# ACDSLab/MPPI-Generic

Measured on AMD Instinct MI355X. Metric: MPPI iters/sec (KxT rollouts), higher is better.
Workload: dtype f32; 1 GPU; Cartpole (CartpoleDynamics + CartpoleQuadraticCost, examples/cartpole_example.cu config) VanillaMPPI optimisation iteration, T=100, dt=0.02, lambda=0.25, sigma=5, Philox noise fused in the rollout kernel, K=16384 rollouts per GPU; rollouts_per_gpu=16384, global_rollouts=16384, parallelism=K-sharded x1, exchange=none

## Files before the change

### include/mppi_amd/dynamics/cartpole/cartpole_dynamics.hpp

```cpp
#ifndef MPPI_AMD_CARTPOLE_DYNAMICS_HPP_
#define MPPI_AMD_CARTPOLE_DYNAMICS_HPP_

#include "mppi_amd/plugin/dynamics.hpp"

struct CartpoleDynamicsParams : public DynamicsParams
{
  enum class StateIndex : int
  {
    POS_X = 0,
    VEL_X,
    THETA,
    THETA_DOT,
    NUM_STATES
  };
  enum class ControlIndex : int
  {
    FORCE = 0,
    NUM_CONTROLS
  };
  enum class OutputIndex : int
  {
    POS_X = 0,
    VEL_X,
    THETA,
    THETA_DOT,
    NUM_OUTPUTS
  };
  float cart_mass = 1.0f;
  float pole_mass = 1.0f;
  float pole_length = 1.0f;

  CartpoleDynamicsParams() = default;
  CartpoleDynamicsParams(float cart_mass, float pole_mass, float pole_length)
    : cart_mass(cart_mass), pole_mass(pole_mass), pole_length(pole_length){};
};

using namespace MPPI_internal;

class CartpoleDynamics : public Dynamics<CartpoleDynamics, CartpoleDynamicsParams>
{
public:
  static constexpr bool MPPI_BARRIER_FREE_STEP = true;
  using PARENT_CLASS = Dynamics<CartpoleDynamics, CartpoleDynamicsParams>;
  CartpoleDynamics(float cart_mass = 1.0f, float pole_mass = 1.0f, float pole_length = 1.0f, hipStream_t stream = 0)
    : PARENT_CLASS(stream)
  {
    this->params_ = CartpoleDynamicsParams(cart_mass, pole_mass, pole_length);
  }

  static const char* getDynamicsModelName()
  {
    return "Cartpole Model";
  }
  __host__ __device__ float getCartMass()
  {
    return this->params_.cart_mass;
  };
  __host__ __device__ float getPoleMass()
  {
    return this->params_.pole_mass;
  };
  __host__ __device__ float getPoleLength()
  {
    return this->params_.pole_length;
  };
  __host__ __device__ float getGravity()
  {
    return gravity_;
  }

  __device__ inline void computeDynamics(float* state, float* control, float* state_der, float* theta = nullptr)
  {
    float theta_n = angle_utils::normalizeAngleBounded(state[2]);
    float sin_theta, cos_theta;
    mppi::det::sincos(theta_n, &sin_theta, &cos_theta);
    float theta_dot = state[3];
    float force = control[0];
    float m_c = this->params_.cart_mass;
    float m_p = this->params_.pole_mass;
    float l_p = this->params_.pole_length;

    state_der[0] = state[1];
    const float den = m_c + m_p * SQ(sin_theta);
    float r_x, r_th;
    mppi::det::rcp_benign2(den, l_p * den, &r_x, &r_th);
    state_der[1] = r_x * (force + m_p * sin_theta * (l_p * SQ(theta_dot) + gravity_ * cos_theta));
    state_der[2] = theta_dot;
    state_der[3] =
        r_th *
        (-force * cos_theta - m_p * l_p * SQ(theta_dot) * cos_theta * sin_theta - (m_c + m_p) * gravity_ * sin_theta);
  }

protected:
  const float gravity_ = 9.81;
};

#endif
```

### include/mppi_amd/engine/rollout_pipeline_kernel.hpp

```cpp
#ifndef MPPI_AMD_ROLLOUT_PIPELINE_KERNEL_HPP_
#define MPPI_AMD_ROLLOUT_PIPELINE_KERNEL_HPP_

#include <type_traits>
#include "rollout_kernel.hpp"
#include "merge_wave.hpp"
#include "kernarg_view.hpp"

namespace mppi
{
namespace kernels
{
constexpr int PIPE_ROLES = 3;
__host__ __device__ constexpr int pipeRingSteps(int output_dim)
{
  return output_dim <= 8 ? 32 : (output_dim <= 16 ? 16 : 8);
}

template <class DYN_T, class COST_T, class SAMPLING_T>
__host__ inline size_t pipelineSharedBytes(const DYN_T& dyn, const COST_T& cost, const SAMPLING_T& smp, int bz,
                                           bool fold_z = false)
{
  const int slots = fold_z ? 64 : 64 * bz;
  const int rings = fold_z ? 1 : bz;
  size_t n = 0;
  n += calcClassSharedMemSize(&dyn, slots);
  n += calcClassSharedMemSize(&cost, slots);
  n += calcClassSharedMemSize(&smp, slots);
  n += sizeof(float) * 2 * math::nearest_multiple_4(slots);
  n += sizeof(float) * (size_t)rings * pipeRingSteps(DYN_T::OUTPUT_DIM) *
       (DYN_T::OUTPUT_DIM + (smp.rows_global_d_ ? DYN_T::CONTROL_DIM : 0)) * 64;
  n += sizeof(int) * 4 * 4 * rings;
  n += sizeof(float) * math::nearest_multiple_4(smp.params_.num_timesteps * DYN_T::CONTROL_DIM);
  return n;
}

typedef volatile __attribute__((address_space(3))) int* lds_counter_t;
typedef int pipe_int4 __attribute__((ext_vector_type(4)));
typedef volatile __attribute__((address_space(3))) pipe_int4* lds_counter4_t;

__device__ inline void pipeWait(lds_counter_t ctr, const int need, int& cached)
{
  if (cached >= need)
    return;
  int v = __builtin_amdgcn_readfirstlane(*ctr);
  while (v < need)
  {
    __builtin_amdgcn_s_sleep(1);
    v = __builtin_amdgcn_readfirstlane(*ctr);
  }
  cached = v;
  __builtin_amdgcn_fence(__ATOMIC_ACQUIRE, "workgroup");
}
__device__ inline void pipePublish(lds_counter_t ctr, const int value, const int lane)
{
  __builtin_amdgcn_fence(__ATOMIC_RELEASE, "workgroup");
  if (lane == 0)
    *ctr = value;
}
__device__ inline void pipePublishLds(lds_counter_t ctr, const int value, const int lane)
{
  asm volatile("" ::: "memory");
  if (lane == 0)
    *ctr = value;
  asm volatile("" ::: "memory");
}
#if defined(MPPI_PIPE_TIMING)
constexpr int PIPE_TIMING_BLOCKS = 256, PIPE_TIMING_WAVES = 24, PIPE_TIMING_SLOTS = 8;
static __device__ unsigned long long g_pipe_timing[PIPE_TIMING_BLOCKS * PIPE_TIMING_WAVES * PIPE_TIMING_SLOTS];
struct PipeTimer
{
  unsigned long long acc[PIPE_TIMING_SLOTS] = {};
  unsigned long long t0 = 0;
  __device__ inline void start()
  {
    t0 = __builtin_amdgcn_s_memtime();
  }
  __device__ inline void stop(const int slot)
  {
    const unsigned long long t1 = __builtin_amdgcn_s_memtime();
    acc[slot] += t1 - t0;
    t0 = t1;
  }
  __device__ inline void trip(const int block, const int kind, const int trip_idx, const int lane, const unsigned long long v) const
  {
    if (block < PIPE_TIMING_BLOCKS && lane == 0 && trip_idx < 4 * PIPE_TIMING_SLOTS && kind < 5)
      g_pipe_timing[(block * PIPE_TIMING_WAVES + 4 + 4 * kind) * PIPE_TIMING_SLOTS + trip_idx] = v;
  }
  __device__ inline void flush(const int block, const int wave, const int lane) const
  {
    if (block < PIPE_TIMING_BLOCKS && wave < PIPE_TIMING_WAVES && lane == 0)
      for (int i = 0; i < PIPE_TIMING_SLOTS; i++)
        g_pipe_timing[(block * PIPE_TIMING_WAVES + wave) * PIPE_TIMING_SLOTS + i] = acc[i];
  }
};
#define PIPE_T(x) x
#else
#define PIPE_T(x)
#endif

constexpr int PIPE_SAMPLERS = 2;
__host__ __device__ constexpr int pipelineBlockX(int bz, bool fold_z)
{
  return (bz == 1 || fold_z) ? 64 * (2 + PIPE_SAMPLERS) : 64 * PIPE_ROLES;
}

template <class DYN_T, class COST_T, class SAMPLING_T, int BZ, bool DRAW_IN_LOOP, bool FOLD_Z = false, bool ROWS_HBM = false,
          bool STREAM_MERGE = false>
__global__ void __launch_bounds__(pipelineBlockX(BZ, FOLD_Z) * (FOLD_Z ? 1 : BZ))
    rolloutPipelineKernel(DYN_T dynamics_obj, COST_T costs_obj, SAMPLING_T sampling_obj, const RolloutArgs args)
{
  static_assert(!STREAM_MERGE || (BZ == 1 && !FOLD_Z && !ROWS_HBM && DRAW_IN_LOOP), "STREAM_MERGE: one system, plain draw, LDS rows");
  static_assert(!FOLD_Z || 64 % BZ == 0, "systems must divide the wave");
  constexpr int BX = FOLD_Z ? 64 / BZ : 64;
  constexpr int WZ = FOLD_Z ? 1 : BZ;
  constexpr bool PAIR_DRAW = FOLD_Z && DRAW_IN_LOOP && BZ == 2 && DYN_T::CONTROL_DIM == 2;
  constexpr int WX = pipelineBlockX(BZ, FOLD_Z);
  constexpr int NS = WX / 64 - 2;
  __builtin_assume(__builtin_amdgcn_workgroup_size_x() == WX);
  __builtin_assume(__builtin_amdgcn_workgroup_size_y() == 1);
  __builtin_assume(__builtin_amdgcn_workgroup_size_z() == WZ);
  __builtin_assume(__builtin_amdgcn_workitem_id_x() < WX);
  __builtin_assume(__builtin_amdgcn_workitem_id_y() == 0);
  __builtin_assume(__builtin_amdgcn_workitem_id_z() < WZ);

  PIPE_T(PipeTimer tm; tm.start(); const unsigned long long t_entry = wall_clock64();)
  DYN_T* dynamics = &dynamics_obj;
  COST_T* costs = &costs_obj;
  SAMPLING_T* sampling = &sampling_obj;
  constexpr int S = DYN_T::STATE_DIM, C = DYN_T::CONTROL_DIM, O = DYN_T::OUTPUT_DIM;
  constexpr int PIPE_RING = pipeRingSteps(O);
  constexpr int SLOTS = BX * BZ;
  constexpr int NTHREADS = WX * WZ;
  constexpr bool SMP_CONSTRAINS = !DYN_T::CONSTRAINTS_DEPEND_ON_STATE;

  const int tid_x = (int)__builtin_amdgcn_workitem_id_x();
  const int wave_x = __builtin_amdgcn_readfirstlane(tid_x >> 6);
  const int role = wave_x < PIPE_ROLES ? wave_x : 0;
  const int smp_id = wave_x < PIPE_ROLES ? 0 : wave_x - PIPE_ROLES + 1;
  const int lane = tid_x & 63;
  const int thread_idx = FOLD_Z ? lane % BX : lane;
  const int thread_idz = FOLD_Z ? lane / BX : (int)__builtin_amdgcn_workitem_id_z();
  const int ring_z = FOLD_Z ? 0 : thread_idz;
  const int block_idx = (int)blockIdx.x;
  const int global_idx = BX * block_idx + thread_idx;
  const int shared_idx = BX * thread_idz + thread_idx;
  const int distribution_idx = thread_idz;
  sampling->setNoiseStream(distribution_idx);
  const int tid_flat = tid_x + WX * ring_z;
  const int num_timesteps = args.num_timesteps;
  const int num_rollouts = args.num_rollouts;
  const float dt = args.dt;
  const bool valid = global_idx < num_rollouts;
  const int nrows = min(BX, num_rollouts - BX * block_idx);

  extern __shared__ __attribute__((aligned(16))) char smem_raw[];
  float* theta_s_shared = reinterpret_cast<float*>(smem_raw);
  float* theta_c_shared = theta_s_shared + calcClassSharedMemSize(dynamics, SLOTS) / (int)sizeof(float);
  float* theta_d_lds = theta_c_shared + calcClassSharedMemSize(costs, SLOTS) / (int)sizeof(float);
  float* theta_d_shared = theta_d_lds;
  if constexpr (ROWS_HBM)
  {
    theta_d_shared = sampling->blockRows(theta_d_lds, (int)blockIdx.x, SLOTS);
    sampling->setStagingBase(theta_d_lds);
  }
  constexpr int F = O + (ROWS_HBM ? C : 0);
  float* cost_s = theta_d_lds + calcClassSharedMemSize(sampling, SLOTS) / (int)sizeof(float);
  float* w_s = cost_s + math::nearest_multiple_4(SLOTS);
  float* ring_all = w_s + math::nearest_multiple_4(SLOTS);
  float* ring = ring_all + (size_t)ring_z * PIPE_RING * F * 64;
  lds_counter_t counters =
      (lds_counter_t)(reinterpret_cast<int*>(ring_all + (size_t)WZ * PIPE_RING * F * 64) + 16 * ring_z);
  float* mean_row_s = ring_all + (size_t)WZ * PIPE_RING * F * 64 + 16 * WZ;
  lds_counter_t smp_prog = counters + 0;
  lds_counter_t smp_prog1 = counters + 1;
  lds_counter_t cost_prog = counters + 2;
  lds_counter_t dyn_prog = counters + 4;
  static_assert(NS <= 2, "one spare counter");

  sampling->setThreadMapping(shared_idx, BX, BZ);

  float x[S], x_next[S], xdot[S], u[C], y[O];
  int crash_status = 0;
#pragma unroll
  for (int i = 0; i < S; i++)
  {
    x[i] = 0.0f;
    xdot[i] = 0.0f;
    x_next[i] = 0.0f;
  }
#pragma unroll
  for (int i = 0; i < C; i++)
    u[i] = 0.0f;
#pragma unroll
  for (int i = 0; i < O; i++)
    y[i] = 0.0f;
  constexpr int SMP_STEPS = 4;
  constexpr int TRIP_COLS = SMP_STEPS * C;
  constexpr int TRIP_GROUPS = TRIP_COLS / MERGE_COLS;
  typedef float merge_f4 __attribute__((ext_vector_type(4)));
  MergeTails mt;
  merge_f4 vq[STREAM_MERGE ? TRIP_GROUPS : 1][MERGE_LANE_RECORDS];
  typedef float merge_f2 __attribute__((ext_vector_type(2)));
  merge_f2 tailq[MERGE_LANE_RECORDS];
  const int TC_all = num_timesteps * C;
  auto load_trip_columns = [&](const int t) {
    if constexpr (STREAM_MERGE)
    {
      static_assert(MERGE_COLS == 4, "the transposed copy is laid out in column quads");
#pragma unroll
      for (int g = 0; g < TRIP_GROUPS; g++)
      {
        const int col0 = t * C + MERGE_COLS * g;
#pragma unroll
        for (int i = 0; i < MERGE_LANE_RECORDS; i++)
        {
          const int b = lane + 64 * i;
          const bool ok = b < args.prev_num_records && col0 < TC_all;
          vq[g][i] = *reinterpret_cast<const merge_f4*>(args.prev_records_t_d +
                                                        ((size_t)(ok ? col0 >> 2 : 0) * args.prev_num_records + (ok ? b : 0)) * 4);
        }
      }
    }
  };
  auto sampler_trip = [&](const int t, auto first_trip) {
    constexpr int QUADS = C;
    float zq[4 * QUADS];
    if (DRAW_IN_LOOP)
    {
#pragma unroll
      for (int q = 0; q < QUADS; q++)
        sampling->drawQuad(global_idx, t * C / 4 + q, &zq[4 * q]);
    }
    PIPE_T(if (decltype(first_trip)::value && smp_id == 0) tm.trip(block_idx, 4, 1, lane, __builtin_amdgcn_s_memtime() - tm.t0);)
    float mu[TRIP_COLS];
    if constexpr (STREAM_MERGE)
    {
      if constexpr (decltype(first_trip)::value)
      {
#pragma unroll
        for (int q = 0; q < 4 * QUADS; q++)
          asm volatile("" : "+v"(zq[q]));
        __builtin_amdgcn_sched_barrier(0);
        float rho_b[MERGE_LANE_RECORDS], eta_b[MERGE_LANE_RECORDS], eta2_b[MERGE_LANE_RECORDS];
#pragma unroll
        for (int i = 0; i < MERGE_LANE_RECORDS; i++)
        {
          const bool ok = lane + 64 * i < args.prev_num_records;
          rho_b[i] = ok ? tailq[i].x : INFINITY;
          eta_b[i] = ok ? tailq[i].y : 0.0f;
          eta2_b[i] = 0.0f;
        }
        mergeTails<false>(rho_b, eta_b, eta2_b, (float)(1.0 / (double)args.lambda), mt);
      }
      PIPE_T(if (decltype(first_trip)::value && smp_id == 0) tm.trip(block_idx, 4, 2, lane, __builtin_amdgcn_s_memtime() - tm.t0);)
#pragma unroll
      for (int g = 0; g < TRIP_GROUPS; g++)
      {
        float v[MERGE_LANE_RECORDS][MERGE_COLS], tot[MERGE_COLS];
#pragma unroll
        for (int i = 0; i < MERGE_LANE_RECORDS; i++)
        {
          const bool ok = lane + 64 * i < args.prev_num_records;
          v[i][0] = ok ? vq[g][i].x : 0.0f;
          v[i][1] = ok ? vq[g][i].y : 0.0f;
          v[i][2] = ok ? vq[g][i].z : 0.0f;
          v[i][3] = ok ? vq[g][i].w : 0.0f;
        }
        mergeColumns(mt.s, v, tot);
#pragma unroll
        for (int c = 0; c < MERGE_COLS; c++)
        {
          mu[MERGE_COLS * g + c] = tot[c] / mt.eta_f;
          if (t * C + MERGE_COLS * g + c < TC_all)
            mean_row_s[t * C + MERGE_COLS * g + c] = mu[MERGE_COLS * g + c];
        }
      }
      PIPE_T(if (decltype(first_trip)::value && smp_id == 0) tm.trip(block_idx, 4, 3, lane, __builtin_amdgcn_s_memtime() - tm.t0);)
      load_trip_columns(t + SMP_STEPS * NS);
    }
#pragma unroll
    for (int s2 = 0; s2 < SMP_STEPS; s2++)
    {
      if (t + s2 < num_timesteps)
      {
        if constexpr (STREAM_MERGE)
          sampling->template shapeControlSampleMean<FOLD_Z>(global_idx, t + s2, distribution_idx, &zq[s2 * C], &mu[s2 * C], u);
        else if (DRAW_IN_LOOP)
          sampling->template shapeControlSample<FOLD_Z>(global_idx, t + s2, distribution_idx, &zq[s2 * C], u);
        else
          sampling->template readControlSample<FOLD_Z>(global_idx, t + s2, distribution_idx, u, theta_d_shared, 1, 0, y);
        if (SMP_CONSTRAINS)
          dynamics->enforceConstraints(x, u);
        sampling->writeControlSample(global_idx, t + s2, distribution_idx, u, theta_d_shared, 1, 0, y);
      }
    }
    PIPE_T(if (decltype(first_trip)::value && smp_id == 0) tm.trip(block_idx, 4, 4, lane, __builtin_amdgcn_s_memtime() - tm.t0);)
  };
  constexpr bool EARLY_FIRST_TRIP = DRAW_IN_LOOP && !PAIR_DRAW;
  static_assert(!STREAM_MERGE || EARLY_FIRST_TRIP, "STREAM_MERGE: the record tails are merged inside the early first trip");
  if constexpr (STREAM_MERGE)
  {
    if (role == 0)
    {
      const float* tails_t = args.prev_records_t_d + (size_t)TC_all * args.prev_num_records;
#pragma unroll
      for (int i = 0; i < MERGE_LANE_RECORDS; i++)
      {
        const int b = lane + 64 * i;
        tailq[i] = *reinterpret_cast<const merge_f2*>(tails_t + 2 * (b < args.prev_num_records ? b : 0));
      }
      load_trip_columns(SMP_STEPS * smp_id);
      asm volatile("" ::: "memory");
      PIPE_T(if (smp_id == 0) tm.trip(block_idx, 4, 0, lane, __builtin_amdgcn_s_memtime() - tm.t0);)
    }
  }
  if (EARLY_FIRST_TRIP && role == 0 && SMP_STEPS * smp_id < num_timesteps)
    sampler_trip(SMP_STEPS * smp_id, std::true_type{});
#pragma unroll
  for (int i = 0; i < S; i++)
    x[i] = args.init_x_d[S * thread_idz + i];

  if (lane == 0 && wave_x == 0)
  {
    *smp_prog = 0;
    *dyn_prog = 0;
    *cost_prog = 0;
    *smp_prog1 = 0;
  }
  __syncthreads();

  dynamics->initializeDynamics(x, u, y, theta_s_shared, 0.0f, dt);
  sampling->initializeDistributions(y, 0.0f, dt, theta_d_shared);
  costs->initializeCosts(y, u, theta_c_shared, 0.0f, dt);
  __syncthreads();

  float running_cost = 0.0f;
  float* row = sampling->sampleRow(theta_d_shared, shared_idx);
  PIPE_T(tm.stop(3);)

  if (role == 0 && PAIR_DRAW)
  {
    constexpr int STEPS = 8 / C;
    lds_counter_t my_prog = smp_id == 0 ? smp_prog : smp_prog1;
    for (int t = STEPS * smp_id; t < num_timesteps; t += STEPS * NS)
    {
      float zq[4], e[8];
      if (sampling->independentNoise())
      {
        sampling->drawQuad(global_idx, t * C / 4, &e[0]);
        sampling->drawQuad(global_idx, t * C / 4 + 1, &e[4]);
      }
      else
      {
        sampling->drawQuad(global_idx, t * C / 4 + thread_idz, zq);
#pragma unroll
        for (int l = 0; l < 4; l++)
        {
          const unsigned v = __float_as_uint(zq[l]);
          auto r = __builtin_amdgcn_permlane32_swap(v, v, false, false);
          e[l] = __uint_as_float(r[0]);
          e[4 + l] = __uint_as_float(r[1]);
        }
      }
#pragma unroll
      for (int s2 = 0; s2 < STEPS; s2++)
      {
        if (t + s2 < num_timesteps)
        {
          sampling->template shapeControlSample<FOLD_Z>(global_idx, t + s2, distribution_idx, &e[s2 * C], u);
          if (SMP_CONSTRAINS)
            dynamics->enforceConstraints(x, u);
          sampling->writeControlSample(global_idx, t + s2, distribution_idx, u, theta_d_shared, 1, 0, y);
        }
      }
      pipePublish(my_prog, min(t + STEPS, num_timesteps), lane);
    }
  }
  else if (role == 0)
  {
    constexpr int STEPS = SMP_STEPS;
    lds_counter_t my_prog = smp_id == 0 ? smp_prog : smp_prog1;
    auto publish = [&](const int value) {
      if constexpr (ROWS_HBM)
        pipePublish(my_prog, value, lane);
      else
        pipePublishLds(my_prog, value, lane);
    };
    int t = STEPS * smp_id;
    if (EARLY_FIRST_TRIP && t < num_timesteps)
    {
      publish(min(t + STEPS, num_timesteps));
      t += STEPS * NS;
    }
    for (; t < num_timesteps; t += STEPS * NS)
    {
      sampler_trip(t, std::false_type{});
      publish(min(t + STEPS, num_timesteps));
      PIPE_T(if (smp_id == 0) { const unsigned long long ts0 = tm.t0; tm.stop(0); tm.trip(block_idx, 3, t / (STEPS * NS), lane, tm.t0 - ts0); })
    }
    PIPE_T(tm.stop(0);)
  }
  else if (role == 1)
  {
    auto dyn_step = [&](float* xc, float* xn, int t, const float* u_in) {
#pragma unroll
      for (int i = 0; i < C; i++)
        u[i] = u_in[i];
      if (!SMP_CONSTRAINS)
      {
        dynamics->enforceConstraints(xc, u);
#pragma unroll
        for (int i = 0; i < C; i++)
          row[t * C + i] = u[i];
      }
      dynamics->step(xc, xn, xdot, u, y, theta_s_shared, t, dt);
      float* slot = ring + (size_t)(t % PIPE_RING) * F * 64 + lane;
#pragma unroll
      for (int i = 0; i < O; i++)
        slot[i * 64] = y[i];
      if constexpr (ROWS_HBM)
      {
#pragma unroll
        for (int i = 0; i < C; i++)
          slot[(O + i) * 64] = u[i];
      }
    };
    int seen_smp = 0, seen_smp1 = 0, seen_cost = 0;
    int t = 0;
    pipe_int4 ahead = { 0, 0, 0, 0 };
    auto look_ahead = [&]() { ahead = *(lds_counter4_t)counters; };
    auto need = [&](lds_counter_t ctr, int& cached, const int ahead_value, const int n) {
      if (cached >= n)
        return;
      cached = max(cached, __builtin_amdgcn_readfirstlane(ahead_value));
      if (cached >= n)
        __builtin_amdgcn_fence(__ATOMIC_ACQUIRE, "workgroup");
      else
        pipeWait(ctr, n, cached);
    };
    auto wait_trip = [&](const int tp, const int n) {
      if (NS == 2 && (tp & 4))
        need(smp_prog1, seen_smp1, ahead.y, n);
      else
        need(smp_prog, seen_smp, ahead.x, n);
    };
    auto wait_ring = [&](const int n) { need(cost_prog, seen_cost, ahead.z, n); };
    float unext[4 * C];
    auto prefetch = [&](const int tp) {
      if (tp < num_timesteps)
      {
        wait_trip(tp, min(tp + 4, num_timesteps));
#pragma unroll
        for (int j = 0; j < 4 * C; j++)
          unext[j] = (tp * C + j < num_timesteps * C) ? row[tp * C + j] : 0.0f;
      }
    };
    if constexpr (ROWS_HBM)
      prefetch(0);
    if constexpr (!ROWS_HBM && NS == 2)
    {
      for (; t + 7 < num_timesteps; t += 8)
      {
        need(smp_prog, seen_smp, ahead.x, t + 4);
        need(smp_prog1, seen_smp1, ahead.y, t + 8);
        PIPE_T(const unsigned long long tw0 = tm.t0; tm.stop(1); tm.trip(block_idx, 0, t / 8, lane, tm.t0 - tw0);)
        wait_ring(t + 8 - PIPE_RING);
        PIPE_T(const unsigned long long tw1 = tm.t0; tm.stop(2); tm.trip(block_idx, 1, t / 8, lane, tm.t0 - tw1);)
        float ubuf[8 * C];
#pragma unroll
        for (int j = 0; j < 8 * C; j++)
          ubuf[j] = row[t * C + j];
        dyn_step(x, x_next, t, &ubuf[0]);
        dyn_step(x_next, x, t + 1, &ubuf[C]);
        dyn_step(x, x_next, t + 2, &ubuf[2 * C]);
        dyn_step(x_next, x, t + 3, &ubuf[3 * C]);
        dyn_step(x, x_next, t + 4, &ubuf[4 * C]);
        dyn_step(x_next, x, t + 5, &ubuf[5 * C]);
        dyn_step(x, x_next, t + 6, &ubuf[6 * C]);
        look_ahead();
        dyn_step(x_next, x, t + 7, &ubuf[7 * C]);
        pipePublishLds(dyn_prog, t + 8, lane);
        PIPE_T(const unsigned long long tw2 = tm.t0; tm.stop(0); tm.trip(block_idx, 2, t / 8, lane, tm.t0 - tw2);)
      }
    }
    for (; t + 3 < num_timesteps; t += 4)
    {
      if constexpr (!ROWS_HBM)
        wait_trip(t, t + 4);
      PIPE_T(tm.stop(1);)
      wait_ring(t + 4 - PIPE_RING);
      PIPE_T(tm.stop(2);)
      float ubuf[4 * C];
      if constexpr (ROWS_HBM)
      {
#pragma unroll
        for (int j = 0; j < 4 * C; j++)
          ubuf[j] = unext[j];
        prefetch(t + 4);
      }
      else
      {
#pragma unroll
        for (int j = 0; j < 4 * C; j++)
          ubuf[j] = row[t * C + j];
      }
      dyn_step(x, x_next, t, &ubuf[0]);
      dyn_step(x_next, x, t + 1, &ubuf[C]);
      dyn_step(x, x_next, t + 2, &ubuf[2 * C]);
      look_ahead();
      dyn_step(x_next, x, t + 3, &ubuf[3 * C]);
      pipePublishLds(dyn_prog, t + 4, lane);
      PIPE_T(tm.stop(0);)
    }
    if (t < num_timesteps)
    {
      const int hi = num_timesteps;
      if constexpr (!ROWS_HBM)
        wait_trip(t, hi);
      wait_ring(hi - PIPE_RING);
      float ubuf[4 * C];
#pragma unroll
      for (int j = 0; j < 4 * C; j++)
        ubuf[j] = ROWS_HBM ? unext[j] : ((t * C + j < num_timesteps * C) ? row[t * C + j] : 0.0f);
      dyn_step(x, x_next, t, &ubuf[0]);
      if (t + 1 < num_timesteps)
        dyn_step(x_next, x, t + 1, &ubuf[C]);
      if (t + 2 < num_timesteps)
        dyn_step(x, x_next, t + 2, &ubuf[2 * C]);
      pipePublishLds(dyn_prog, hi, lane);
      PIPE_T(tm.stop(0);)
    }
  }
  else if (role == 2)
  {
    int seen_dyn = 0;
    auto cost_step = [&](const int tt) {
      const float* slot = ring + (size_t)(tt % PIPE_RING) * F * 64 + lane;
#pragma unroll
      for (int i = 0; i < O; i++)
        y[i] = slot[i * 64];
#pragma unroll
      for (int i = 0; i < C; i++)
        u[i] = ROWS_HBM ? slot[(O + i) * 64] : row[tt * C + i];
      running_cost += costs->computeRunningCost(y, u, tt, theta_c_shared, &crash_status) +
                      sampling->template computeLikelihoodRatioCost<FOLD_Z, STREAM_MERGE>(u, theta_d_shared, global_idx, tt,
                                                                                          distribution_idx, args.lambda,
                                                                                          args.alpha, mean_row_s);
    };
    int t = 0;
    for (; t + 3 < num_timesteps; t += 4)
    {
      pipeWait(dyn_prog, t + 4, seen_dyn);
      PIPE_T(tm.stop(1);)
      cost_step(t);
      cost_step(t + 1);
      cost_step(t + 2);
      cost_step(t + 3);
      pipePublishLds(cost_prog, t + 4, lane);
      PIPE_T(tm.stop(0);)
    }
    if (t < num_timesteps)
    {
      pipeWait(dyn_prog, num_timesteps, seen_dyn);
      PIPE_T(tm.stop(1);)
      for (int tt = t; tt < num_timesteps; tt++)
        cost_step(tt);
      pipePublishLds(cost_prog, num_timesteps, lane);
      PIPE_T(tm.stop(0);)
    }
  }
  __syncthreads();
  PIPE_T(tm.stop(4);)

  const bool writer = (role == 2);
  const float terminal = costs->terminalCost(y, theta_c_shared);
  blockSoftminEpilogue<SAMPLING_T, C, BX, BZ, NTHREADS>(sampling, args, terminal, running_cost, writer, valid, global_idx,
                                                        shared_idx, thread_idz, tid_flat, block_idx, nrows,
                                                        theta_d_shared, cost_s, w_s);
  PIPE_T(tm.stop(5); tm.acc[6] = t_entry; tm.acc[7] = wall_clock64(); tm.flush(block_idx, wave_x + 4 * ring_z, lane);)
}


template <class SAMPLING_T>
__host__ __device__ inline int samplerGrdBytes(const SAMPLING_T* smp)
{
  return ((smp->getGrdSharedSizeBytes() + 15) / 16) * 16;
}

#if !defined(MPPI_PIPE_REP_NS)
#define MPPI_PIPE_REP_NS 2
#define MPPI_PIPE_REP_NC 2
#endif
constexpr int PIPE_REP_SAMPLERS = MPPI_PIPE_REP_NS;
constexpr int PIPE_REP_COSTS = MPPI_PIPE_REP_NC;

template <class DYN_T, class COST_T, class SAMPLING_T>
__host__ inline size_t pipelineRepSharedBytes(const DYN_T& dyn, const COST_T& cost, const SAMPLING_T& smp, int ring)
{
  const int slots = 64;
  size_t n = 0;
  n += calcClassSharedMemSize(&dyn, slots);
  n += calcClassSharedMemSize(&cost, slots);
  n += calcClassSharedMemSize(&smp, slots) - samplerGrdBytes(&smp);
  const size_t ring_bytes = sizeof(float) * (size_t)ring * (DYN_T::OUTPUT_DIM + (smp.rows_global_d_ ? DYN_T::CONTROL_DIM : 0)) * 64;
  n += ring_bytes > (size_t)samplerGrdBytes(&smp) ? ring_bytes : (size_t)samplerGrdBytes(&smp);
  n += sizeof(float) * 4 * math::nearest_multiple_4(slots);
  n += sizeof(int) * 4 * (replicated_lanes<DYN_T>::value + PIPE_REP_SAMPLERS + 1);
  return n;
}

template <class DYN_T, class COST_T, class SAMPLING_T>
__host__ inline int pipelineRepRingSteps(const DYN_T& dyn, const COST_T& cost, const SAMPLING_T& smp, size_t max_lds)
{
  for (int ring = 32; ring >= 4; ring >>= 1)
    if (pipelineRepSharedBytes(dyn, cost, smp, ring) <= max_lds)
      return ring;
  return 0;
}

template <class T>
__device__ inline void vgprResident(T& obj)
{
  static_assert(sizeof(T) % 4 == 0, "whole words");
  uint32_t* w = reinterpret_cast<uint32_t*>(&obj);
#pragma unroll
  for (int i = 0; i < (int)(sizeof(T) / 4); i++)
    asm volatile("" : "+v"(w[i]));
}

template <class DYN_T, class COST_T, class SAMPLING_T, bool DRAW_IN_LOOP, bool ROWS_HBM = false>
#if !defined(MPPI_PIPE_REP_MIN_WAVES)
#define MPPI_PIPE_REP_MIN_WAVES 2
#endif
#if MPPI_PIPE_REP_MIN_WAVES > 0
#define MPPI_PIPE_REP_BOUNDS(n) __launch_bounds__(n, MPPI_PIPE_REP_MIN_WAVES)
#else
#define MPPI_PIPE_REP_BOUNDS(n) __launch_bounds__(n)
#endif
__global__ void MPPI_PIPE_REP_BOUNDS(64 * (replicated_lanes<DYN_T>::value + PIPE_REP_SAMPLERS + PIPE_REP_COSTS))
    rolloutPipelineRepKernel(DYN_T dynamics_obj, COST_T costs_obj, SAMPLING_T sampling_obj, const RolloutArgs args,
                             const int ring_steps)
{
  constexpr int BX = 64;
  constexpr int REP = replicated_lanes<DYN_T>::value;
  static_assert(REP > 1 && 64 % REP == 0, "this variant is for replicated-lane dynamics");
  constexpr int DW = BX * REP / 64;
  constexpr int NS = PIPE_REP_SAMPLERS, NC = PIPE_REP_COSTS;
  constexpr int NWAVES = DW + NS + NC;
  constexpr int NTHREADS = 64 * NWAVES;
  constexpr int PER_WAVE = 64 / REP;
  __builtin_assume(__builtin_amdgcn_workgroup_size_x() == NTHREADS);
  __builtin_assume(__builtin_amdgcn_workgroup_size_y() == 1);
  __builtin_assume(__builtin_amdgcn_workgroup_size_z() == 1);
  __builtin_assume(__builtin_amdgcn_workitem_id_x() < NTHREADS);
  __builtin_assume(__builtin_amdgcn_workitem_id_y() == 0);
  __builtin_assume(__builtin_amdgcn_workitem_id_z() == 0);

  DYN_T* dynamics = &dynamics_obj;
  COST_T* costs = &costs_obj;
  SAMPLING_T* sampling = &sampling_obj;
  constexpr int S = DYN_T::STATE_DIM, C = DYN_T::CONTROL_DIM, O = DYN_T::OUTPUT_DIM;
  constexpr int SLOTS = BX;
  constexpr bool SMP_CONSTRAINS = !DYN_T::CONSTRAINTS_DEPEND_ON_STATE;

  const int tid_x = (int)__builtin_amdgcn_workitem_id_x();
  const int wave = __builtin_amdgcn_readfirstlane(tid_x >> 6);
  const int lane = tid_x & 63;
  const bool is_dyn = wave < DW;
  const bool is_sampler = !is_dyn && wave < DW + NS;
  const int helper_id = is_dyn ? 0 : (is_sampler ? wave - DW : wave - DW - NS);
  const int thread_idx = is_dyn ? wave * PER_WAVE + (lane % PER_WAVE) : lane;
  const int rep_lane = is_dyn ? lane / PER_WAVE : 0;
  const int block_idx = (int)blockIdx.x;
  const int global_idx = BX * block_idx + thread_idx;
  const int shared_idx = thread_idx;
  const int num_timesteps = args.num_timesteps;
  const int num_rollouts = args.num_rollouts;
  const float dt = args.dt;
  const bool valid = global_idx < num_rollouts;
  const int nrows = min(BX, num_rollouts - BX * block_idx);
  const int ring_mask = ring_steps - 1;

  extern __shared__ __attribute__((aligned(16))) char smem_raw[];
  float* theta_s_shared = reinterpret_cast<float*>(smem_raw);
  float* theta_c_shared = theta_s_shared + calcClassSharedMemSize(dynamics, SLOTS) / (int)sizeof(float);
  float* theta_d_lds = theta_c_shared + calcClassSharedMemSize(costs, SLOTS) / (int)sizeof(float);
  float* theta_d_shared = theta_d_lds;
  if constexpr (ROWS_HBM)
  {
    theta_d_shared = sampling->blockRows(theta_d_lds, block_idx, SLOTS);
    sampling->setStagingBase(theta_d_lds);
  }
  constexpr int F = O + (ROWS_HBM ? C : 0);
  float* ring = theta_d_lds + (calcClassSharedMemSize(sampling, SLOTS) - samplerGrdBytes(sampling)) / (int)sizeof(float);
  const int overlay_floats = max(ring_steps * F * 64, samplerGrdBytes(sampling) / (int)sizeof(float));
  float* cost_s = ring + overlay_floats;
  float* w_s = cost_s + math::nearest_multiple_4(SLOTS);
  float* relay_cost = w_s + math::nearest_multiple_4(SLOTS);
  int* relay_status = reinterpret_cast<int*>(relay_cost + math::nearest_multiple_4(SLOTS));
  lds_counter_t counters = (lds_counter_t)(relay_status + math::nearest_multiple_4(SLOTS));
  static_assert(NS <= 2, "the sampler counters share a 16-byte group with the cost counter");
  lds_counter_t cost_prog = counters + 2;

  sampling->setThreadMapping(shared_idx, BX);

  float x[S], x_next[S], xdot[S], u[C], y[O];
  int crash_status = 0;
#pragma unroll
  for (int i = 0; i < S; i++)
  {
    x[i] = args.init_x_d[i];
    xdot[i] = 0.0f;
    x_next[i] = 0.0f;
  }
#pragma unroll
  for (int i = 0; i < C; i++)
    u[i] = 0.0f;
#pragma unroll
  for (int i = 0; i < O; i++)
    y[i] = 0.0f;
  if (tid_x < 4 + DW)
    counters[tid_x] = 0;
  __syncthreads();

  dynamics->initializeDynamics(x, u, y, theta_s_shared, 0.0f, dt);
  sampling->initializeDistributions(y, 0.0f, dt, theta_d_shared);
  costs->initializeCosts(y, u, theta_c_shared, 0.0f, dt);
  __syncthreads();

  float running_cost = 0.0f;
  float* row = sampling->sampleRow(theta_d_shared, shared_idx);
  constexpr int STEPS = (C % 2 == 0) ? 2 : 4;

  if (is_sampler)
  {
    constexpr int QUADS = STEPS * C / 4;
    lds_counter_t smp_prog = counters + helper_id;
    PIPE_T(PipeTimer tm; tm.start();)
    for (int t = STEPS * helper_id; t < num_timesteps; t += STEPS * NS)
    {
      float zq[4 * QUADS];
      if (DRAW_IN_LOOP)
      {
#pragma unroll
        for (int q = 0; q < QUADS; q++)
          sampling->drawQuad(global_idx, t * C / 4 + q, &zq[4 * q]);
      }
#pragma unroll
      for (int s2 = 0; s2 < STEPS; s2++)
      {
        if (t + s2 < num_timesteps)
        {
          if (DRAW_IN_LOOP)
            sampling->shapeControlSample(global_idx, t + s2, 0, &zq[s2 * C], u);
          else
            sampling->readControlSample(global_idx, t + s2, 0, u, theta_d_shared, 1, 0, y);
          if (SMP_CONSTRAINS)
            dynamics->enforceConstraints(x, u);
          sampling->writeControlSample(global_idx, t + s2, 0, u, theta_d_shared, 1, 0, y);
        }
      }
      if constexpr (ROWS_HBM)
        pipePublish(smp_prog, min(t + STEPS, num_timesteps), lane);
      else
        pipePublishLds(smp_prog, min(t + STEPS, num_timesteps), lane);
    }
    PIPE_T(tm.stop(0); tm.flush(block_idx, wave, lane);)
  }
  else if (is_dyn)
  {
    lds_counter_t my_prog = counters + 4 + wave;
    auto dyn_step = [&](float* xc, float* xn, int t, const float* u_in) {
#pragma unroll
      for (int i = 0; i < C; i++)
        u[i] = u_in[i];
      if (!SMP_CONSTRAINS)
      {
        dynamics->enforceConstraints(xc, u);
#pragma unroll
        for (int i = 0; i < C; i++)
          row[t * C + i] = u[i];
      }
      dynamics->step(xc, xn, xdot, u, y, theta_s_shared, t, dt);
      {
        float* slot = ring + (size_t)(t & ring_mask) * F * 64 + thread_idx;
#pragma unroll
        for (int i = 0; i < O; i++)
          slot[i * 64] = y[i];
        if constexpr (ROWS_HBM)
        {
#pragma unroll
          for (int i = 0; i < C; i++)
            slot[(O + i) * 64] = u[i];
        }
      }
    };
    int seen_smp[NS], seen_cost = 0;
#pragma unroll
    for (int q = 0; q < NS; q++)
      seen_smp[q] = 0;
    pipe_int4 ahead = { 0, 0, 0, 0 };
    auto look_ahead = [&]() { ahead = *(lds_counter4_t)counters; };
    auto need = [&](lds_counter_t ctr, int& cached, const int ahead_value, const int n) {
      if (cached >= n)
        return;
      cached = max(cached, __builtin_amdgcn_readfirstlane(ahead_value));
      if (cached >= n)
        __builtin_amdgcn_fence(__ATOMIC_ACQUIRE, "workgroup");
      else
        pipeWait(ctr, n, cached);
    };
    auto wait_samples = [&](const int t, const int n) {
      if constexpr (NS == 1)
        need(counters, seen_smp[0], ahead.x, n);
      else
      {
        const int owner = (t / STEPS) % NS;
        if (owner == 0)
          need(counters, seen_smp[0], ahead.x, n);
        else
          need(counters + 1, seen_smp[NS - 1], ahead.y, n);
      }
    };
    int t = 0;
    PIPE_T(PipeTimer tm; tm.start();)
    float unext[2 * C];
    auto prefetch = [&](const int tp) {
      if (tp < num_timesteps)
      {
        wait_samples(tp, min(tp + 2, num_timesteps));
#pragma unroll
        for (int j = 0; j < 2 * C; j++)
          unext[j] = (tp * C + j < num_timesteps * C) ? row[tp * C + j] : 0.0f;
      }
    };
    if constexpr (ROWS_HBM)
      prefetch(0);
    for (; t + 1 < num_timesteps; t += 2)
    {
      if constexpr (!ROWS_HBM)
        wait_samples(t, t + 2);
      PIPE_T(tm.stop(1);)
      need(cost_prog, seen_cost, ahead.z, t + 2 - ring_steps);
      PIPE_T(tm.stop(2);)
      float ubuf[2 * C];
      if constexpr (ROWS_HBM)
      {
#pragma unroll
        for (int j = 0; j < 2 * C; j++)
          ubuf[j] = unext[j];
        prefetch(t + 2);
      }
      else
      {
#pragma unroll
        for (int j = 0; j < 2 * C; j++)
          ubuf[j] = row[t * C + j];
      }
      dyn_step(x, x_next, t, &ubuf[0]);
      look_ahead();
      dyn_step(x_next, x, t + 1, &ubuf[C]);
      pipePublishLds(my_prog, t + 2, lane);
      PIPE_T(tm.stop(0);)
    }
    PIPE_T(tm.flush(block_idx, wave, lane);)
    if (t < num_timesteps)
    {
      if constexpr (!ROWS_HBM)
        wait_samples(t, num_timesteps);
      need(cost_prog, seen_cost, ahead.z, num_timesteps - ring_steps);
      float ubuf[C];
#pragma unroll
      for (int j = 0; j < C; j++)
        ubuf[j] = ROWS_HBM ? unext[j] : row[t * C + j];
      dyn_step(x, x_next, t, &ubuf[0]);
      pipePublishLds(my_prog, num_timesteps, lane);
    }
  }
  else
  {
    constexpr bool COST_VIEW = MPPI_KERNARG_RELOAD && MPPI_COST_KERNARG_VIEW && kernarg_viewable<COST_T>::value;
    constexpr size_t COST_OFFSET = KernargLayout<DYN_T, COST_T>::template offset<1>();
    COST_T costs_v = *costs;
    if constexpr (!COST_VIEW)
      vgprResident(costs_v);
    COST_T* costs_w = &costs_v;
    int seen_dyn[DW], seen_cost = 0;
#pragma unroll
    for (int w = 0; w < DW; w++)
      seen_dyn[w] = 0;
    int status_guess = 0;
    PIPE_T(PipeTimer tm; tm.start();)
    for (int t = 2 * helper_id; t < num_timesteps; t += 2 * NC)
    {
      const int hi = min(t + 2, num_timesteps);
#pragma unroll
      for (int w = 0; w < DW; w++)
        pipeWait(counters + 4 + w, hi, seen_dyn[w]);
      PIPE_T(tm.stop(1);)
      float yb[2][O], ub[2][C];
#pragma unroll
      for (int q = 0; q < 2; q++)
      {
        const int tt = min(t + q, num_timesteps - 1);
        const float* slot = ring + (size_t)(tt & ring_mask) * F * 64 + lane;
#pragma unroll
        for (int i = 0; i < O; i++)
          yb[q][i] = slot[i * 64];
#pragma unroll
        for (int i = 0; i < C; i++)
          ub[q][i] = ROWS_HBM ? slot[(O + i) * 64] : row[tt * C + i];
      }
      PIPE_T(tm.stop(3);)
      float cq[2] = { 0.0f, 0.0f };
      auto evaluate = [&](int status) {
        if constexpr (COST_VIEW)
          costs_w = kernargObject<COST_T>(kernargBase(), COST_OFFSET);
#pragma unroll
        for (int q = 0; q < 2; q++)
        {
          if (t + q < num_timesteps)
            cq[q] = costs_w->computeRunningCost(yb[q], ub[q], t + q, theta_c_shared, &status) +
                    sampling->computeLikelihoodRatioCost(ub[q], theta_d_shared, global_idx, t + q, 0, args.lambda, args.alpha);
        }
        return status;
      };
      int status_out = evaluate(status_guess);
      PIPE_T(tm.stop(0);)
      if (t > 0)
      {
        pipeWait(cost_prog, t, seen_cost);
        running_cost = relay_cost[lane];
        crash_status = relay_status[lane];
      }
      PIPE_T(tm.stop(2);)
      if (__builtin_amdgcn_ballot_w64(crash_status != status_guess) != 0ull)
      {
        status_out = evaluate(crash_status);
        PIPE_T(tm.stop(4);)
      }
      running_cost += cq[0];
      if (t + 1 < num_timesteps)
        running_cost += cq[1];
      crash_status = status_out;
      status_guess = status_out;
      relay_cost[lane] = running_cost;
      relay_status[lane] = crash_status;
      pipePublishLds(cost_prog, hi, lane);
      PIPE_T(tm.stop(5);)
    }
    PIPE_T(tm.flush(block_idx, wave, lane);)
  }
  __syncthreads();

  const bool writer = !is_dyn && !is_sampler && helper_id == 0;
  if (writer)
  {
    running_cost = relay_cost[lane];
    const float* slot = ring + (size_t)((num_timesteps - 1) & ring_mask) * F * 64 + lane;
#pragma unroll
    for (int i = 0; i < O; i++)
      y[i] = slot[i * 64];
  }
  const float terminal = costs->terminalCost(y, theta_c_shared);
  blockSoftminEpilogue<SAMPLING_T, C, BX, 1, NTHREADS>(sampling, args, terminal, running_cost, writer, valid, global_idx,
                                                       shared_idx, 0, tid_x, block_idx, nrows, theta_d_shared, cost_s, w_s);
}

}
}

#endif
```

### include/mppi_amd/plugin/dynamics.hpp

```cpp
#ifndef MPPI_AMD_PLUGIN_DYNAMICS_HPP_
#define MPPI_AMD_PLUGIN_DYNAMICS_HPP_

#include <cfloat>
#include <hip/hip_runtime.h>
#include "mppi_amd/plugin/managed.hpp"
#include "mppi_amd/plugin/math_utils.hpp"
#include "mppi_amd/plugin/parallel_utils.hpp"
#include "mppi_amd/plugin/host_arrays.hpp"

#ifndef E_INDEX
#define E_INDEX(ENUM, enum_val) static_cast<int>(ENUM::enum_val)
#endif
#ifndef S_INDEX
#define S_IND_CLASS(CLASS, enum_val) E_INDEX(CLASS::StateIndex, enum_val)
#define S_INDEX(enum_val) S_IND_CLASS(PARENT_CLASS::DYN_PARAMS_T, enum_val)
#endif
#ifndef C_INDEX
#define C_IND_CLASS(CLASS, enum_val) E_INDEX(CLASS::ControlIndex, enum_val)
#define C_INDEX(enum_val) C_IND_CLASS(PARENT_CLASS::DYN_PARAMS_T, enum_val)
#endif
#ifndef O_INDEX
#define O_IND_CLASS(CLASS, enum_val) E_INDEX(CLASS::OutputIndex, enum_val)
#define O_INDEX(enum_val) O_IND_CLASS(PARENT_CLASS::DYN_PARAMS_T, enum_val)
#endif

struct DynamicsParams
{
  enum class StateIndex : int
  {
    POS_X = 0,
    NUM_STATES
  };
  enum class ControlIndex : int
  {
    VEL_X = 0,
    NUM_CONTROLS
  };
  enum class OutputIndex : int
  {
    POS_X = 0,
    NUM_OUTPUTS
  };
};

namespace MPPI_internal
{
template <class CLASS_T, class PARAMS_T>
class Dynamics : public mppi::Managed
{
public:
  static const int STATE_DIM = S_IND_CLASS(PARAMS_T, NUM_STATES);
  static const int CONTROL_DIM = C_IND_CLASS(PARAMS_T, NUM_CONTROLS);
  static const int OUTPUT_DIM = O_IND_CLASS(PARAMS_T, NUM_OUTPUTS);
  typedef CLASS_T DYN_T;
  typedef PARAMS_T DYN_PARAMS_T;
  typedef mppi::host::Array<STATE_DIM> state_array;
  typedef mppi::host::Array<CONTROL_DIM> control_array;
  typedef mppi::host::Array<OUTPUT_DIM> output_array;

  Dynamics(hipStream_t stream = 0)
  {
    bindToStream(stream);
    for (int i = 0; i < CONTROL_DIM; i++)
    {
      control_rngs_[i].x = -FLT_MAX;
      control_rngs_[i].y = FLT_MAX;
      control_deadband_[i] = 0.0f;
      zero_control_[i] = 0.0f;
    }
  }

  hipError_t GPUSetup()
  {
    CLASS_T* derived = static_cast<CLASS_T*>(this);
    if (!GPUMemStatus_)
    {
      hipError_t e = Managed::GPUSetup(derived, &model_d_);
      if (e != hipSuccess)
        return e;
    }
    return derived->paramsToDevice();
  }
  hipError_t freeCudaMem()
  {
    hipError_t e = hipSuccess;
    if (GPUMemStatus_)
    {
      e = hipFree(model_d_);
      GPUMemStatus_ = false;
      model_d_ = nullptr;
    }
    return e;
  }
  hipError_t paramsToDevice(bool synchronize = true)
  {
    if (!GPUMemStatus_)
      return hipSuccess;
    hipError_t e = hipMemcpyAsync(&model_d_->params_, &params_, sizeof(PARAMS_T), hipMemcpyHostToDevice, stream_);
    if (e == hipSuccess)
      e = hipMemcpyAsync(&model_d_->control_rngs_, &control_rngs_, CONTROL_DIM * sizeof(float2),
                         hipMemcpyHostToDevice, stream_);
    if (e == hipSuccess)
      e = hipMemcpyAsync(&model_d_->control_deadband_, &control_deadband_, CONTROL_DIM * sizeof(float),
                         hipMemcpyHostToDevice, stream_);
    if (e == hipSuccess)
      e = hipMemcpyAsync(&model_d_->zero_control_, &zero_control_, CONTROL_DIM * sizeof(float), hipMemcpyHostToDevice,
                         stream_);
    if (e == hipSuccess && synchronize)
      e = hipStreamSynchronize(stream_);
    return e;
  }
  void setParams(const PARAMS_T& params)
  {
    params_ = params;
    (void)paramsToDevice();
  }
  __host__ __device__ PARAMS_T getParams() const
  {
    return params_;
  }
  void setControlRanges(const float2* control_rngs)
  {
    for (int i = 0; i < CONTROL_DIM; i++)
      control_rngs_[i] = control_rngs[i];
    (void)paramsToDevice();
  }
  void setControlDeadbands(const float* control_deadband)
  {
    for (int i = 0; i < CONTROL_DIM; i++)
      control_deadband_[i] = control_deadband[i];
    (void)paramsToDevice();
  }

  void enforceConstraints(state_array& state, control_array& control);
  void step(state_array& state, state_array& next_state, state_array& state_der, control_array& control,
            output_array& output, const float t, const float dt);
  void printState(const float* state) const
  {
    printf("State:");
    for (int i = 0; i < STATE_DIM; i++)
      printf(" %f", state[i]);
    printf("\n");
  }

  __device__ inline void initializeDynamics(float* state, float* control, float* output, float* theta_s, float t_0,
                                            float dt)
  {
    static_cast<CLASS_T*>(this)->stateToOutput(state, output);
  }

  static constexpr bool CONSTRAINTS_DEPEND_ON_STATE = false;
  static constexpr bool BASE_CONSTRAINTS = true;

  __device__ inline void enforceConstraints(float* state, float* control)
  {
    int i, p_index, step;
    mppi::p1::getParallel1DIndex<mppi::p1::Parallel1Dir::THREAD_Y>(p_index, step);
    for (i = p_index; i < CONTROL_DIM; i += step)
    {
      if (fabsf(control[i]) < this->control_deadband_[i])
      {
        control[i] = this->zero_control_[i];
      }
      else
      {
        control[i] += this->control_deadband_[i] * -mppi::math::sign(control[i]);
      }
      control[i] = fminf(fmaxf(this->control_rngs_[i].x, control[i]), this->control_rngs_[i].y);
    }
  }

  __device__ inline void computeKinematics(float* state, float* state_der)
  {
  }

  __device__ inline void computeStateDeriv(float* state, float* control, float* state_der, float* theta_s)
  {
    CLASS_T* derived = static_cast<CLASS_T*>(this);
    if (__builtin_amdgcn_workitem_id_y() == 0)
    {
      derived->computeKinematics(state, state_der);
    }
    derived->computeDynamics(state, control, state_der, theta_s);
  }

  __device__ inline void updateState(float* state, float* next_state, float* state_der, const float dt)
  {
    int i, p_index, step;
    mppi::p1::getParallel1DIndex<mppi::p1::Parallel1Dir::THREAD_Y>(p_index, step);
#if defined(__HIP_DEVICE_COMPILE__)
    if (STATE_DIM % 2 == 0 && step == 1)
    {
      typedef float f32x2 __attribute__((ext_vector_type(2)));
#pragma unroll
      for (i = 0; i + 1 < STATE_DIM; i += 2)
      {
        const f32x2 x = { state[i], state[i + 1] };
        const f32x2 d = { state_der[i], state_der[i + 1] };
        const f32x2 inc = d * f32x2{ dt, dt };
        const f32x2 n = x + inc;
        next_state[i] = n.x;
        next_state[i + 1] = n.y;
      }
      return;
    }
#endif
    for (i = p_index; i < STATE_DIM; i += step)
    {
      next_state[i] = state[i] + state_der[i] * dt;
    }
  }

  __device__ inline void step(float* state, float* next_state, float* state_der, float* control, float* output,
                              float* theta_s, const float t, const float dt)
  {
    CLASS_T* derived = static_cast<CLASS_T*>(this);
    derived->computeStateDeriv(state, control, state_der, theta_s);
    mppi::lane_sync();
    derived->updateState(state, next_state, state_der, dt);
    mppi::lane_sync();
    derived->stateToOutput(next_state, output);
  }

  __device__ inline void stateToOutput(const float* __restrict__ state, float* __restrict__ output)
  {
    int p_index, step;
    mppi::p1::getParallel1DIndex<mppi::p1::Parallel1Dir::THREAD_Y>(p_index, step);
    for (int i = p_index; i < OUTPUT_DIM && i < STATE_DIM; i += step)
    {
      output[i] = state[i];
    }
  }
  __device__ inline void outputToState(const float* __restrict__ output, float* __restrict__ state)
  {
    int p_index, step;
    mppi::p1::getParallel1DIndex<mppi::p1::Parallel1Dir::THREAD_Y>(p_index, step);
    for (int i = p_index; i < OUTPUT_DIM && i < STATE_DIM; i += step)
    {
      state[i] = output[i];
    }
  }

  CLASS_T* model_d_ = nullptr;

  PARAMS_T params_;
  float2 control_rngs_[CONTROL_DIM];
  float control_deadband_[CONTROL_DIM];
  float zero_control_[CONTROL_DIM];
};
}

#endif
```

Measured before the change: 42270 MPPI iters/s.

## Split cartpole step between dynamics and cost pipeline roles

Adds an opt-in split-step interface for dynamics models. The cartpole dynamics role now computes only the pole angle and angular-velocity update, and passes next theta_dot, sin and cos through a 3-float ring slot instead of 4 outputs. The cost role then finishes the cart position and velocity update from that carry before computing the running cost. This moves work off the serial dynamics critical path and shrinks LDS ring traffic. In exchange the cost role does more work and must keep its own copy of the state in sync.

```diff
diff --git a/include/mppi_amd/dynamics/cartpole/cartpole_dynamics.hpp b/include/mppi_amd/dynamics/cartpole/cartpole_dynamics.hpp
--- a/include/mppi_amd/dynamics/cartpole/cartpole_dynamics.hpp
+++ b/include/mppi_amd/dynamics/cartpole/cartpole_dynamics.hpp
@@ -91,6 +91,51 @@
         (-force * cos_theta - m_p * l_p * SQ(theta_dot) * cos_theta * sin_theta - (m_c + m_p) * gravity_ * sin_theta);
   }
 
+  using SPLIT_STEP_CLASS = CartpoleDynamics;
+  static constexpr int SPLIT_CARRY = 3;
+
+  __device__ inline void stepCore(const float* state, float* next_state, const float* control, float* carry, const float dt)
+  {
+    float theta_n = angle_utils::normalizeAngleBounded(state[2]);
+    float sin_theta, cos_theta;
+    mppi::det::sincos(theta_n, &sin_theta, &cos_theta);
+    float theta_dot = state[3];
+    float force = control[0];
+    float m_c = this->params_.cart_mass;
+    float m_p = this->params_.pole_mass;
+    float l_p = this->params_.pole_length;
+    const float den = m_c + m_p * SQ(sin_theta);
+    const float r_th = mppi::det::rcp_benign(l_p * den);
+    const float theta_dd =
+        r_th *
+        (-force * cos_theta - m_p * l_p * SQ(theta_dot) * cos_theta * sin_theta - (m_c + m_p) * gravity_ * sin_theta);
+    next_state[2] = state[2] + theta_dot * dt;
+    next_state[3] = theta_dot + theta_dd * dt;
+    carry[0] = next_state[3];
+    carry[1] = sin_theta;
+    carry[2] = cos_theta;
+  }
+
+  __device__ inline void stepComplete(float* state, const float* control, const float* carry, float* output, const float dt)
+  {
+    const float sin_theta = carry[1], cos_theta = carry[2];
+    float theta_dot = state[3];
+    float force = control[0];
+    float m_c = this->params_.cart_mass;
+    float m_p = this->params_.pole_mass;
+    float l_p = this->params_.pole_length;
+    const float den = m_c + m_p * SQ(sin_theta);
+    const float r_x = mppi::det::rcp_benign(den);
+    const float x_dd = r_x * (force + m_p * sin_theta * (l_p * SQ(theta_dot) + gravity_ * cos_theta));
+    state[0] = state[0] + state[1] * dt;
+    state[1] = state[1] + x_dd * dt;
+    state[2] = state[2] + theta_dot * dt;
+    state[3] = carry[0];
+#pragma unroll
+    for (int i = 0; i < 4; i++)
+      output[i] = state[i];
+  }
+
 protected:
   const float gravity_ = 9.81;
 };
diff --git a/include/mppi_amd/engine/rollout_pipeline_kernel.hpp b/include/mppi_amd/engine/rollout_pipeline_kernel.hpp
--- a/include/mppi_amd/engine/rollout_pipeline_kernel.hpp
+++ b/include/mppi_amd/engine/rollout_pipeline_kernel.hpp
@@ -5,6 +5,7 @@
 #include "rollout_kernel.hpp"
 #include "merge_wave.hpp"
 #include "kernarg_view.hpp"
+#include "mppi_amd/plugin/dynamics.hpp"
 
 namespace mppi
 {
@@ -14,6 +15,15 @@
 __host__ __device__ constexpr int pipeRingSteps(int output_dim)
 {
   return output_dim <= 8 ? 32 : (output_dim <= 16 ? 16 : 8);
+}
+
+template <class DYN_T>
+__host__ __device__ constexpr int pipeRingOutputFloats()
+{
+  if constexpr (split_step<DYN_T>::value)
+    return DYN_T::SPLIT_CARRY;
+  else
+    return DYN_T::OUTPUT_DIM;
 }
 
 template <class DYN_T, class COST_T, class SAMPLING_T>
@@ -28,7 +38,7 @@
   n += calcClassSharedMemSize(&smp, slots);
   n += sizeof(float) * 2 * math::nearest_multiple_4(slots);
   n += sizeof(float) * (size_t)rings * pipeRingSteps(DYN_T::OUTPUT_DIM) *
-       (DYN_T::OUTPUT_DIM + (smp.rows_global_d_ ? DYN_T::CONTROL_DIM : 0)) * 64;
+       (pipeRingOutputFloats<DYN_T>() + (smp.rows_global_d_ ? DYN_T::CONTROL_DIM : 0)) * 64;
   n += sizeof(int) * 4 * 4 * rings;
   n += sizeof(float) * math::nearest_multiple_4(smp.params_.num_timesteps * DYN_T::CONTROL_DIM);
   return n;
@@ -163,7 +173,9 @@
     theta_d_shared = sampling->blockRows(theta_d_lds, (int)blockIdx.x, SLOTS);
     sampling->setStagingBase(theta_d_lds);
   }
-  constexpr int F = O + (ROWS_HBM ? C : 0);
+  constexpr bool SPLIT = split_step<DYN_T>::value;
+  constexpr int RY = pipeRingOutputFloats<DYN_T>();
+  constexpr int F = RY + (ROWS_HBM ? C : 0);
   float* cost_s = theta_d_lds + calcClassSharedMemSize(sampling, SLOTS) / (int)sizeof(float);
   float* w_s = cost_s + math::nearest_multiple_4(SLOTS);
   float* ring_all = w_s + math::nearest_multiple_4(SLOTS);
@@ -413,16 +425,27 @@
         for (int i = 0; i < C; i++)
           row[t * C + i] = u[i];
       }
-      dynamics->step(xc, xn, xdot, u, y, theta_s_shared, t, dt);
       float* slot = ring + (size_t)(t % PIPE_RING) * F * 64 + lane;
-#pragma unroll
-      for (int i = 0; i < O; i++)
-        slot[i * 64] = y[i];
+      if constexpr (SPLIT)
+      {
+        float carry[RY];
+        dynamics->stepCore(xc, xn, u, carry, dt);
+#pragma unroll
+        for (int i = 0; i < RY; i++)
+          slot[i * 64] = carry[i];
+      }
+      else
+      {
+        dynamics->step(xc, xn, xdot, u, y, theta_s_shared, t, dt);
+#pragma unroll
+        for (int i = 0; i < O; i++)
+          slot[i * 64] = y[i];
+      }
       if constexpr (ROWS_HBM)
       {
 #pragma unroll
         for (int i = 0; i < C; i++)
-          slot[(O + i) * 64] = u[i];
+          slot[(RY + i) * 64] = u[i];
       }
     };
     int seen_smp = 0, seen_smp1 = 0, seen_cost = 0;
@@ -537,11 +560,22 @@
     auto cost_step = [&](const int tt) {
       const float* slot = ring + (size_t)(tt % PIPE_RING) * F * 64 + lane;
 #pragma unroll
-      for (int i = 0; i < O; i++)
-        y[i] = slot[i * 64];
-#pragma unroll
       for (int i = 0; i < C; i++)
-        u[i] = ROWS_HBM ? slot[(O + i) * 64] : row[tt * C + i];
+        u[i] = ROWS_HBM ? slot[(RY + i) * 64] : row[tt * C + i];
+      if constexpr (SPLIT)
+      {
+        float carry[RY];
+#pragma unroll
+        for (int i = 0; i < RY; i++)
+          carry[i] = slot[i * 64];
+        dynamics->stepComplete(x, u, carry, y, dt);
+      }
+      else
+      {
+#pragma unroll
+        for (int i = 0; i < O; i++)
+          y[i] = slot[i * 64];
+      }
       running_cost += costs->computeRunningCost(y, u, tt, theta_c_shared, &crash_status) +
                       sampling->template computeLikelihoodRatioCost<FOLD_Z, STREAM_MERGE>(u, theta_d_shared, global_idx, tt,
                                                                                           distribution_idx, args.lambda,
diff --git a/include/mppi_amd/plugin/dynamics.hpp b/include/mppi_amd/plugin/dynamics.hpp
--- a/include/mppi_amd/plugin/dynamics.hpp
+++ b/include/mppi_amd/plugin/dynamics.hpp
@@ -250,4 +250,16 @@
 };
 }
 
-#endif
+namespace mppi
+{
+template <class T, class = void>
+struct split_step : std::false_type
+{
+};
+template <class T>
+struct split_step<T, std::void_t<typename T::SPLIT_STEP_CLASS>> : std::is_same<typename T::SPLIT_STEP_CLASS, T>
+{
+};
+}
+
+#endif
```

New measurement: 45780 MPPI iters/s (median of 6 runs). 8.3% higher.
